# hritikbharucha/Custom_Porechop_ABI

Measured on AMD Instinct MI355X. Metric: reads/sec trimmed (100k ONT reads x 50 adapter pairs), higher is better.
Workload: dtype int32

## Files before the change

custom_porechop_abi_amd/csrc/pcabi_dp.h:

```cpp
#pragma once

#ifndef PCABI_ROW_FENCE
#define PCABI_ROW_FENCE 1
#endif
#ifndef PCABI_TAB_PD
#define PCABI_TAB_PD 0
#endif
#ifndef PCABI_TAB_PD_LONG
#define PCABI_TAB_PD_LONG 1
#endif

#include <stdint.h>
#include <algorithm>

#ifdef __HIPCC__
#define PCABI_HD __host__ __device__ __forceinline__
#else
#define PCABI_HD inline
#endif

namespace pcabi {

constexpr int NEG = -(1 << 28);

// ... 1158 lines not shown
template <typename TabRow>
struct ShiftRow {
    TabRow t;
    int32_t d;
    PCABI_HD int32_t operator()(int s) const { return addw(t(s), d); }
    PCABI_HD void quad(int q, int32_t *dst) const {
        t.quad(q, dst);
        for (int k = 0; k < 4; ++k) dst[k] = addw(dst[k], d);
    }
};
}

template <int RPL, int PD = PCABI_TAB_PD>
struct LaneShift {
    using Y = pk::LayS<RPL>;
    LanePacked<RPL, true, pk::LayT<RPL>, PD> st;
    int32_t kgo;
    int32_t ftop;
    int32_t k_e;
    int32_t k_eR;
    int32_t k_rb;
    int jj, P;

    PCABI_HD void init(int L, const Scoring &sc, int P_, int B) {
        using pk::addw;
        const int off = RPL - L;
        P = P_;
        jj = 0;
        k_e = Y::sc(-sc.ge);
        k_eR = Y::sc(-sc.ge * RPL);
        k_rb = Y::sc(sc.ge * P);
        ftop = Y::sc(-B);
        kgo = Y::sc(sc.go - sc.ge) + ((P - 1) << Y::TB_SH);
        int32_t fs = addw(ftop, kgo);
#pragma unroll
        for (int s = 1; s <= RPL; ++s) {
            fs = addw(fs, k_e);
            st.G[s] = addw(Y::start(off - s), fs);
            st.HK[s] = addw(fs, Y::sc(-1) + Y::TAG1);
        }
        st.bkey = Y::start(-L);
        st.bj = 0;
    }

    PCABI_HD void advance() {
        using pk::addw;
        ++jj;
        kgo -= Y::TAG1;
        ftop = addw(ftop, k_e);
        if (jj == P) {
            const int32_t rb = addw(k_rb, P << Y::TB_SH);
#pragma unroll
            for (int s = 1; s <= RPL; ++s) {
                st.G[s] = addw(st.G[s], rb);
                st.HK[s] = addw(st.HK[s], rb);
            }
            jj = 0;
            kgo += P << Y::TB_SH;
            ftop = addw(ftop, k_rb);
        }
    }

    template <typename TabRow>
    PCABI_HD void column(const TabRow &tab, const int j, const int off) {
        using pk::addw;
        const int32_t kg = vreg(kgo);
        const int32_t top = addw(ftop, kgo);
        int32_t gup = addw(Y::start(j + off), top);
        int32_t vup = Y::SENT;
        int32_t diag = addw(addw(Y::start(j - 1 + off), top), Y::TAG1 - k_e);
        constexpr int NQ = RPL / 4;
        int32_t t[RPL + 2];
// ... 6 lines not shown
#pragma unroll
        for (int s = 1; s <= RPL; ++s) {
            if (PD > 0 && (s & 3) == 1) {
                const int q = (s - 1) / 4 + PD + 1;
                if (q < NQ) tab.quad(q, t + 4 * q + 1);
            }
            int32_t diag_nx = 0;
            if (s < RPL) diag_nx = st.G[s] + (PD > 0 ? t[s + 1] : tab(s + 1));
            const int32_t hn = std::max(st.HK[s], st.G[s]);
            const int32_t vo = gup + Y::kv(s);
            const int32_t vn = std::max(vup, vo);
            const int32_t sn = max3i(diag, vn, hn);
            if (s == RPL) { lv = vn; ls = sn; }
            st.G[s] = (sn & ~Y::TAGM) + kg;
            st.HK[s] = hn;
            gup = st.G[s];
            vup = vn;
            diag = diag_nx;
#if defined(__HIP_DEVICE_COMPILE__)
            if (PCABI_ROW_FENCE > 0 && (s % (PCABI_ROW_FENCE > 0 ? PCABI_ROW_FENCE : 1)) == 0) __builtin_amdgcn_sched_barrier(0);
#endif
        }
        const int32_t corr = addw(std::max(lv, ls & ~Y::TAGM), pk::negw(addw(ftop, k_eR)));
        const bool upd = corr > (st.bkey | ((1 << Y::SC_SH) - 1));
        st.bkey = upd ? corr : st.bkey;
        st.bj = upd ? j : st.bj;
    }

    PCABI_HD void to_layt(const Scoring &sc) {
        using pk::addw;
        using pk::negw;
        const int32_t tagA = kgo - Y::sc(sc.go - sc.ge);
        int32_t cg = addw(negw(addw(ftop, kgo)), Y::sc(sc.go));
        int32_t ch = negw(addw(ftop, tagA + Y::TAG1));
#pragma unroll
        for (int s = 1; s <= RPL; ++s) {
            cg = addw(cg, negw(k_e));
            ch = addw(ch, negw(k_e));
            st.G[s] = addw(st.G[s], cg);
            st.HK[s] = addw(st.HK[s], ch);
        }
    }
};

template <int RPL, int PD = PCABI_TAB_PD, typename ReadFn, typename TabFn>
PCABI_HD Result align_lane_shift(ReadFn &rd, int n, const TabFn &tabfn, int L, const Scoring sc, int P, int B) {
    using Y = pk::LayS<RPL>;
    LaneShift<RPL, PD> ls;
    const int off = RPL - L;
    ls.init(L, sc, P, B);
    int r = rd(1);
#pragma unroll 1
    for (int j = 1; j < n; ++j) {
        const int rn = rd(j + 1);
        ls.advance();
        ls.template column<decltype(tabfn(r))>(tabfn(r), j, off);
        r = rn;
    }
    ls.to_layt(sc);
    auto &st = ls.st;
    const int32_t neg = Y::sc(pk::neg_score(sc));
    st.k_ge = vreg(Y::sc(sc.ge));
    st.k_go = vreg(Y::sc(sc.go));
    st.k_gev = st.k_geh = 0;
    st.k_gex = vreg(Y::sc(sc.ge) + Y::TB1);
    st.k_vo = Y::TB2;
    st.neg2 = neg | Y::TB2;
    st.materialize(L);
    const pk::ShiftRow<decltype(tabfn(r))> row{tabfn(r), Y::sc(sc.ge) + ((127 - Y::TDS) << Y::TB_SH)};
    st.template column<decltype(row), true>(row, n, L, off);
    Best b;
    b.score = st.bscore; b.bi = st.bi; b.bj = st.bj; b.attr = Y::to_std(st.battr, st.bj);
    b.ltype = st.blt; b.trail = st.btrail; b.precd = st.bprec;
    return finish(b, L, n);
}

template <int RPL, bool AFFINE, bool CHUNK = false, typename ReadFn, typename TabFn0, typename TabFn1>
PCABI_HD Result align_lane_packed_long(ReadFn &rd0, ReadFn &rd1, int n, const TabFn0 &tab0, const TabFn1 &tab1,
                                       int L, const Scoring sc, int own_lo = 1, int own_hi = -1) {
    int n_fin;
    Best b = packed_best<RPL, AFFINE, CHUNK, pk::LayL<RPL, 0>, PCABI_TAB_PD_LONG>(rd0, n, tab0, L, sc, own_lo, own_hi,
                                                                                 n_fin);
    const Best bm = packed_best<RPL, AFFINE, CHUNK, pk::LayL<RPL, 1>, PCABI_TAB_PD_LONG>(rd1, n, tab1, L, sc, own_lo,
                                                                                        own_hi, n_fin);
    b.attr |= bm.attr;
    return finish(b, L, n_fin);
}

struct SplitIn {
    int32_t gup, vup;
    int slt, vt, vp;
    int score, bi, lt, trail, prec;
    uint32_t attr;
};

template <int R, bool AFFINE, typename LAY>
struct LaneSplit {
// ... 352 lines not shown
```

custom_porechop_abi_amd/csrc/pcabi_kern.h:

```cpp
#pragma once
#include <hip/hip_runtime.h>

#include <algorithm>
#include <cstdint>
#include <cstdlib>
#include <string>
#include <type_traits>

#include "../../include/pcabi.h"
#include "pcabi_dp.h"

#ifndef PCABI_WAVES
#define PCABI_WAVES 1
#endif

void pcabi_poison(void *p, size_t bytes);
void pcabi_poison_async(void *p, size_t bytes, hipStream_t st);

namespace pcabi_eng {

int fail(int code, const std::string &msg);

#define HIP_TRY(expr)                                                                   \
    do {                                                                                \
// ... 131 lines not shown
        const int c = e / RPL, srow = e % RPL + 1;
        const uint32_t *ap = p.adp_pad + (int64_t)a_local * (RPL / 4);
        auto code = [&](int sl) { return (int)((ap[(sl - 1) / 4] >> (8 * ((sl - 1) & 3))) & 0xFFu); };
        wave_tab[e] = pcabi::pk::sub_key_shift<RPL>(srow, c, code, off, p.sc);
    }
    __syncthreads();
}

template <int RPL>
__device__ __forceinline__ void fill_wave_tab_long(const KParams &p, int a_local, int L, int32_t *wave_tab) {
    const int off = RPL - L;
    const int lane = threadIdx.x & 63;
    const uint32_t *ap = p.adp_pad + (int64_t)a_local * (RPL / 4);
    auto code = [&](int sl) { return (int)((ap[(sl - 1) / 4] >> (8 * ((sl - 1) & 3))) & 0xFFu); };
    for (int e = lane; e < kTabW * RPL; e += 64) {
        const int c = e / RPL, srow = e % RPL + 1;
        wave_tab[e] = pcabi::pk::sub_key<RPL, decltype(code), pcabi::pk::LayL<RPL, 0>>(srow, c, code, off, p.sc);
        wave_tab[kTabW * RPL + e] =
            pcabi::pk::sub_key<RPL, decltype(code), pcabi::pk::LayL<RPL, 1>>(srow, c, code, off, p.sc);
    }
    __syncthreads();
}

template <int RPL, bool AFFINE, int KIND>
__device__ __forceinline__ void run_lane(const KParams &p, int a_local, int64_t w, int64_t out_idx,
                                         int32_t *wave_tab, int64_t tile_off) {
    AdapterRegs<RPL> adp;
    if constexpr (KIND != LONG) adp.load(p.adp_pad + (int64_t)a_local * (RPL / 4));
    const int L = __builtin_amdgcn_readfirstlane(p.adp_len[a_local]);
    if constexpr (KIND == PACKED) fill_wave_tab<RPL>(p, a_local, L, wave_tab);
    if constexpr (KIND == TAGGED) fill_wave_tab<RPL, pcabi::pk::LayT<RPL>>(p, a_local, L, wave_tab);
    if constexpr (KIND == SHIFT) fill_wave_tab_shift<RPL>(p, a_local, L, wave_tab);
    if constexpr (KIND == LONG) fill_wave_tab_long<RPL>(p, a_local, L, wave_tab);
    if (w < 0) return;
    const int n = p.win_len[w];
    pcabi::Result r;
    if (n <= 0) {
        r = empty_result();
    } else {
        WindowReader rd = tile_off >= 0
            ? WindowReader(p.tiles + tile_off + (threadIdx.x & 255), 256, 0)
            : [&] {
                  const uint8_t *b = p.codes + p.win_off[w];
                  const int a0 = (int)((uintptr_t)b & 3);
                  return WindowReader(reinterpret_cast<const uint32_t *>(b - a0), 1, 8 * a0);
              }();
        if constexpr (KIND == PACKED) {
            auto tabfn = [&](int rc) { return LdsRow{wave_tab + rc * RPL}; };
            r = pcabi::align_lane_packed<(RPL <= pcabi::pk::MAX_RPL ? RPL : 4), AFFINE>(rd, n, tabfn, L, p.sc);
        } else if constexpr (KIND == TAGGED) {
            static_assert(RPL <= 32 && AFFINE, "run-tagged layout: affine buckets of <= 32 rows");
            auto tabfn = [&](int rc) { return LdsRow{wave_tab + rc * RPL}; };
            r = pcabi::align_lane_packed<RPL, true, false, pcabi::pk::LayT<RPL>>(rd, n, tabfn, L, p.sc);
        } else if constexpr (KIND == SHIFT) {
            static_assert(RPL <= 32 && AFFINE, "gap-extend frame: affine buckets of <= 32 rows");
            auto tabfn = [&](int rc) { return LdsRow{wave_tab + rc * RPL}; };
            r = pcabi::align_lane_shift<RPL>(rd, n, tabfn, L, p.sc, p.shift_p, p.shift_b);
        } else if constexpr (KIND == LONG) {
            WindowReader rd1 = rd;
            auto tab0 = [&](int rc) { return LdsRow{wave_tab + rc * RPL}; };
// ... 487 lines not shown
```

Baseline: 15.80 million.

## Add 4-column unrolled shift DP path for wave-uniform tiled windows

Adds align_lane_shift4, which reads one packed 32-bit tile word per four read columns and runs four DP columns per loop iteration. Only the first column of each group checks the periodic rebase; the other three use a cheaper step() since P is a multiple of 4. The fast path runs only when every lane in the wave has the same window length and tiled input, so per-column reader overhead and branches go away and loads are prefetched two words ahead. The best-score comparison is also changed to compare extracted scores, and the change adds register pressure and an extra wave-wide ballot check.

```diff
diff --git a/custom_porechop_abi_amd/csrc/pcabi_dp.h b/custom_porechop_abi_amd/csrc/pcabi_dp.h
--- a/custom_porechop_abi_amd/csrc/pcabi_dp.h
+++ b/custom_porechop_abi_amd/csrc/pcabi_dp.h
@@ -1204,16 +1204,16 @@
     int32_t k_rb;
     int jj, P;
 
-    PCABI_HD void init(int L, const Scoring &sc, int P_, int B) {
+    PCABI_HD void init(int L, const Scoring &sc, int P_, int B, int j0 = 0) {
         using pk::addw;
         const int off = RPL - L;
         P = P_;
-        jj = 0;
+        jj = j0;
         k_e = Y::sc(-sc.ge);
         k_eR = Y::sc(-sc.ge * RPL);
         k_rb = Y::sc(sc.ge * P);
-        ftop = Y::sc(-B);
-        kgo = Y::sc(sc.go - sc.ge) + ((P - 1) << Y::TB_SH);
+        ftop = Y::sc(-sc.ge * j0 - B);
+        kgo = Y::sc(sc.go - sc.ge) + ((P - 1 - j0) << Y::TB_SH);
         int32_t fs = addw(ftop, kgo);
 #pragma unroll
         for (int s = 1; s <= RPL; ++s) {
@@ -1225,11 +1225,15 @@
         st.bj = 0;
     }
 
+    PCABI_HD void step() {
+        ++jj;
+        kgo -= Y::TAG1;
+        ftop = pk::addw(ftop, k_e);
+    }
+
     PCABI_HD void advance() {
         using pk::addw;
-        ++jj;
-        kgo -= Y::TAG1;
-        ftop = addw(ftop, k_e);
+        step();
         if (jj == P) {
             const int32_t rb = addw(k_rb, P << Y::TB_SH);
 #pragma unroll
@@ -1282,7 +1286,7 @@
 #endif
         }
         const int32_t corr = addw(std::max(lv, ls & ~Y::TAGM), pk::negw(addw(ftop, k_eR)));
-        const bool upd = corr > (st.bkey | ((1 << Y::SC_SH) - 1));
+        const bool upd = Y::score(corr) > Y::score(st.bkey);
         st.bkey = upd ? corr : st.bkey;
         st.bj = upd ? j : st.bj;
     }
@@ -1303,9 +1307,29 @@
     }
 };
 
+template <int RPL, int PD, typename TabRow>
+PCABI_HD Result shift_last(LaneShift<RPL, PD> &ls, const TabRow &tab, int n, int L, const Scoring &sc) {
+    using Y = pk::LayS<RPL>;
+    ls.to_layt(sc);
+    auto &st = ls.st;
+    const int32_t neg = Y::sc(pk::neg_score(sc));
+    st.k_ge = vreg(Y::sc(sc.ge));
+    st.k_go = vreg(Y::sc(sc.go));
+    st.k_gev = st.k_geh = 0;
+    st.k_gex = vreg(Y::sc(sc.ge) + Y::TB1);
+    st.k_vo = Y::TB2;
+    st.neg2 = neg | Y::TB2;
+    st.materialize(L);
+    const pk::ShiftRow<TabRow> row{tab, Y::sc(sc.ge) + ((127 - Y::TDS) << Y::TB_SH)};
+    st.template column<decltype(row), true>(row, n, L, RPL - L);
+    Best b;
+    b.score = st.bscore; b.bi = st.bi; b.bj = st.bj; b.attr = Y::to_std(st.battr, st.bj);
+    b.ltype = st.blt; b.trail = st.btrail; b.precd = st.bprec;
+    return finish(b, L, n);
+}
+
 template <int RPL, int PD = PCABI_TAB_PD, typename ReadFn, typename TabFn>
 PCABI_HD Result align_lane_shift(ReadFn &rd, int n, const TabFn &tabfn, int L, const Scoring sc, int P, int B) {
-    using Y = pk::LayS<RPL>;
     LaneShift<RPL, PD> ls;
     const int off = RPL - L;
     ls.init(L, sc, P, B);
@@ -1317,22 +1341,37 @@
         ls.template column<decltype(tabfn(r))>(tabfn(r), j, off);
         r = rn;
     }
-    ls.to_layt(sc);
-    auto &st = ls.st;
-    const int32_t neg = Y::sc(pk::neg_score(sc));
-    st.k_ge = vreg(Y::sc(sc.ge));
-    st.k_go = vreg(Y::sc(sc.go));
-    st.k_gev = st.k_geh = 0;
-    st.k_gex = vreg(Y::sc(sc.ge) + Y::TB1);
-    st.k_vo = Y::TB2;
-    st.neg2 = neg | Y::TB2;
-    st.materialize(L);
-    const pk::ShiftRow<decltype(tabfn(r))> row{tabfn(r), Y::sc(sc.ge) + ((127 - Y::TDS) << Y::TB_SH)};
-    st.template column<decltype(row), true>(row, n, L, off);
-    Best b;
-    b.score = st.bscore; b.bi = st.bi; b.bj = st.bj; b.attr = Y::to_std(st.battr, st.bj);
-    b.ltype = st.blt; b.trail = st.btrail; b.precd = st.bprec;
-    return finish(b, L, n);
+    return shift_last<RPL, PD>(ls, tabfn(r), n, L, sc);
+}
+
+template <int RPL, int PD = PCABI_TAB_PD, typename TileFn, typename TabFn>
+PCABI_HD Result align_lane_shift4(const TileFn &tr, int n, const TabFn &tabfn, int L, const Scoring sc, int P, int B) {
+    LaneShift<RPL, PD> ls;
+    const int off = RPL - L;
+    ls.init(L, sc, P, B, -1);
+    const int np = (n - 1) / 4;
+    uint32_t cur = tr(0), nx = tr(1);
+    int j = 1;
+#pragma unroll 1
+    for (int q = 0; q < np; ++q, j += 4) {
+        const uint32_t w = cur;
+        cur = nx;
+        nx = tr(q + 2);
+        ls.advance();
+        ls.template column<decltype(tabfn(0))>(tabfn((int)(w & 0xFFu)), j, off);
+        ls.step();
+        ls.template column<decltype(tabfn(0))>(tabfn((int)((w >> 8) & 0xFFu)), j + 1, off);
+        ls.step();
+        ls.template column<decltype(tabfn(0))>(tabfn((int)((w >> 16) & 0xFFu)), j + 2, off);
+        ls.step();
+        ls.template column<decltype(tabfn(0))>(tabfn((int)(w >> 24)), j + 3, off);
+    }
+#pragma unroll 1
+    for (; j < n; ++j) {
+        ls.advance();
+        ls.template column<decltype(tabfn(0))>(tabfn((int)((cur >> (8 * ((j - 1) & 3))) & 0xFFu)), j, off);
+    }
+    return shift_last<RPL, PD>(ls, tabfn((int)((cur >> (8 * ((n - 1) & 3))) & 0xFFu)), n, L, sc);
 }
 
 template <int RPL, bool AFFINE, bool CHUNK = false, typename ReadFn, typename TabFn0, typename TabFn1>
diff --git a/custom_porechop_abi_amd/csrc/pcabi_kern.h b/custom_porechop_abi_amd/csrc/pcabi_kern.h
--- a/custom_porechop_abi_amd/csrc/pcabi_kern.h
+++ b/custom_porechop_abi_amd/csrc/pcabi_kern.h
@@ -177,6 +177,8 @@
     __syncthreads();
 }
 
+constexpr int kShift4MaxRows = 24;
+
 template <int RPL, bool AFFINE, int KIND>
 __device__ __forceinline__ void run_lane(const KParams &p, int a_local, int64_t w, int64_t out_idx,
                                          int32_t *wave_tab, int64_t tile_off) {
@@ -190,7 +192,20 @@
     if (w < 0) return;
     const int n = p.win_len[w];
     pcabi::Result r;
-    if (n <= 0) {
+    bool uniform = false;
+    if constexpr (KIND == SHIFT) {
+        const int n0 = __builtin_amdgcn_readfirstlane(n);
+        const int P = __builtin_amdgcn_readfirstlane(p.shift_p);
+        if (RPL <= kShift4MaxRows && n0 > 0 && (P & 3) == 0 && __builtin_amdgcn_ballot_w64(n != n0 || tile_off < 0) == 0) {
+            const uint32_t *base = p.tiles + tile_off + (threadIdx.x & 255);
+            auto tr = [&](int q) { return base[(int64_t)q * 256]; };
+            auto tabfn = [&](int rc) { return LdsRow{wave_tab + rc * RPL}; };
+            r = pcabi::align_lane_shift4<RPL>(tr, n0, tabfn, L, p.sc, P, p.shift_b);
+            uniform = true;
+        }
+    }
+    if (uniform) {
+    } else if (n <= 0) {
         r = empty_result();
     } else {
         WindowReader rd = tile_off >= 0
diff --git a/profiles/r08/k_align24_shift4_inner_pass.s b/profiles/r08/k_align24_shift4_inner_pass.s
--- /dev/null
+++ b/profiles/r08/k_align24_shift4_inner_pass.s
@@ -0,0 +1,1008 @@
+	s_mov_b64 s[4:5], 0x400
+.LBB5_25:
+	global_load_dword v62, v[8:9], off
+	s_add_i32 s53, s53, 1
+	s_add_i32 s48, s48, 0xfffe0000
+	s_add_i32 s47, s47, s42
+	s_cmp_lg_u32 s53, s34
+	s_cbranch_scc1 .LBB5_27
+	v_add_u32_e32 v59, s50, v59
+	v_add_u32_e32 v60, s50, v60
+	v_add_u32_e32 v57, s50, v57
+	v_add_u32_e32 v58, s50, v58
+	v_add_u32_e32 v55, s50, v55
+	v_add_u32_e32 v56, s50, v56
+	v_add_u32_e32 v53, s50, v53
+	v_add_u32_e32 v54, s50, v54
+	v_add_u32_e32 v51, s50, v51
+	v_add_u32_e32 v52, s50, v52
+	v_add_u32_e32 v49, s50, v49
+	v_add_u32_e32 v50, s50, v50
+	v_add_u32_e32 v47, s50, v47
+	v_add_u32_e32 v48, s50, v48
+	v_add_u32_e32 v45, s50, v45
+	v_add_u32_e32 v46, s50, v46
+	v_add_u32_e32 v43, s50, v43
+	v_add_u32_e32 v44, s50, v44
+	v_add_u32_e32 v41, s50, v41
+	v_add_u32_e32 v42, s50, v42
+	v_add_u32_e32 v39, s50, v39
+	v_add_u32_e32 v40, s50, v40
+	v_add_u32_e32 v37, s50, v37
+	v_add_u32_e32 v38, s50, v38
+	v_add_u32_e32 v35, s50, v35
+	v_add_u32_e32 v36, s50, v36
+	v_add_u32_e32 v33, s50, v33
+	v_add_u32_e32 v34, s50, v34
+	v_add_u32_e32 v31, s50, v31
+	v_add_u32_e32 v32, s50, v32
+	v_add_u32_e32 v29, s50, v29
+	v_add_u32_e32 v30, s50, v30
+	v_add_u32_e32 v27, s50, v27
+	v_add_u32_e32 v28, s50, v28
+	v_add_u32_e32 v25, s50, v25
+	v_add_u32_e32 v26, s50, v26
+	v_add_u32_e32 v23, s50, v23
+	v_add_u32_e32 v24, s50, v24
+	v_add_u32_e32 v20, s50, v20
+	v_add_u32_e32 v21, s50, v21
+	v_add_u32_e32 v17, s50, v17
+	v_add_u32_e32 v19, s50, v19
+	v_add_u32_e32 v15, s50, v15
+	v_add_u32_e32 v16, s50, v16
+	v_add_u32_e32 v22, s50, v22
+	v_add_u32_e32 v14, s50, v14
+	v_add_u32_e32 v10, s50, v10
+	v_add_u32_e32 v11, s50, v11
+	s_add_i32 s48, s48, s45
+	s_add_i32 s47, s47, s44
+	s_mov_b32 s53, 0
+.LBB5_27:
+	s_waitcnt vmcnt(2)
+	v_and_b32_e32 v63, 0xff, v61
+	v_mad_u32_u24 v63, v63, s52, v18
+	v_mov_b32_e32 v66, s48
+	s_add_i32 s36, s51, 0xfffff400
+	ds_read_b64 v[64:65], v63
+	s_and_b32 s36, s36, 0x1fc00
+	s_add_i32 s10, s47, s48
+	s_add_i32 s11, s51, 0xfffdf800
+	s_sub_i32 s36, s36, s42
+	s_and_b32 s11, s11, 0x1fc00
+	s_add_i32 s36, s10, s36
+	s_add_i32 s36, s36, 0x20000
+	s_add_i32 s10, s10, s11
+	s_waitcnt lgkmcnt(0)
+	v_add_u32_e32 v64, s36, v64
+	v_add_u32_e32 v65, v65, v59
+	v_max_i32_e32 v59, v60, v59
+	s_add_i32 s10, s10, 0xbe0000
+	v_max3_i32 v60, v64, s10, v59
+	v_and_b32_e32 v60, 0xff01ffff, v60
+	v_add_u32_e32 v60, v60, v66
+	ds_read_b32 v64, v63 offset:8
+	v_add_u32_e32 v67, 0xbc0000, v60
+	v_max_i32_e32 v58, v58, v57
+	v_max_i32_e32 v67, s10, v67
+	v_max3_i32 v65, v65, v67, v58
+	s_waitcnt lgkmcnt(0)
+	v_add_u32_e32 v57, v64, v57
+	v_and_b32_e32 v64, 0xff01ffff, v65
+	v_add_u32_e32 v64, v64, v66
+	ds_read_b32 v65, v63 offset:12
+	v_add_u32_e32 v68, 0xba0000, v64
+	v_max_i32_e32 v56, v56, v55
+	v_max_i32_e32 v67, v67, v68
+	v_max3_i32 v57, v57, v67, v56
+	v_and_b32_e32 v57, 0xff01ffff, v57
+	s_waitcnt lgkmcnt(0)
+	v_add_u32_e32 v55, v65, v55
+	v_add_u32_e32 v57, v57, v66
+	ds_read_b32 v65, v63 offset:16
+	v_add_u32_e32 v68, 0xb80000, v57
+	v_max_i32_e32 v54, v54, v53
+	v_max_i32_e32 v67, v67, v68
+	v_max3_i32 v55, v55, v67, v54
+	v_and_b32_e32 v55, 0xff01ffff, v55
+	s_waitcnt lgkmcnt(0)
+	v_add_u32_e32 v53, v65, v53
+	v_add_u32_e32 v55, v55, v66
+	ds_read_b32 v65, v63 offset:20
+	v_add_u32_e32 v68, 0xb60000, v55
+	v_max_i32_e32 v52, v52, v51
+	v_max_i32_e32 v67, v67, v68
+	v_max3_i32 v53, v53, v67, v52
+	v_and_b32_e32 v53, 0xff01ffff, v53
+	s_waitcnt lgkmcnt(0)
+	v_add_u32_e32 v51, v65, v51
+	v_add_u32_e32 v53, v53, v66
+	ds_read_b32 v65, v63 offset:24
+	v_add_u32_e32 v68, 0xb40000, v53
+	v_max_i32_e32 v50, v50, v49
+	v_max_i32_e32 v67, v67, v68
+	v_max3_i32 v51, v51, v67, v50
+	v_and_b32_e32 v51, 0xff01ffff, v51
+	s_waitcnt lgkmcnt(0)
+	v_add_u32_e32 v49, v65, v49
+	v_add_u32_e32 v51, v51, v66
+	ds_read_b32 v65, v63 offset:28
+	v_add_u32_e32 v68, 0xb20000, v51
+	v_max_i32_e32 v48, v48, v47
+	v_max_i32_e32 v67, v67, v68
+	v_max3_i32 v49, v49, v67, v48
+	v_and_b32_e32 v49, 0xff01ffff, v49
+	s_waitcnt lgkmcnt(0)
+	v_add_u32_e32 v47, v65, v47
+	v_add_u32_e32 v49, v49, v66
+	ds_read_b32 v65, v63 offset:32
+	v_add_u32_e32 v68, 0xb00000, v49
+	v_max_i32_e32 v46, v46, v45
+	v_max_i32_e32 v67, v67, v68
+	v_max3_i32 v47, v47, v67, v46
+	v_and_b32_e32 v47, 0xff01ffff, v47
+	s_waitcnt lgkmcnt(0)
+	v_add_u32_e32 v45, v65, v45
+	v_add_u32_e32 v47, v47, v66
+	ds_read_b32 v65, v63 offset:36
+	v_add_u32_e32 v68, 0xae0000, v47
+	v_max_i32_e32 v44, v44, v43
+	v_max_i32_e32 v67, v67, v68
+	v_max3_i32 v45, v45, v67, v44
+	v_and_b32_e32 v45, 0xff01ffff, v45
+	s_waitcnt lgkmcnt(0)
+	v_add_u32_e32 v43, v65, v43
+	v_add_u32_e32 v45, v45, v66
+	ds_read_b32 v65, v63 offset:40
+	v_add_u32_e32 v68, 0xac0000, v45
+	v_max_i32_e32 v42, v42, v41
+	v_max_i32_e32 v67, v67, v68
+	v_max3_i32 v43, v43, v67, v42
+	v_and_b32_e32 v43, 0xff01ffff, v43
+	s_waitcnt lgkmcnt(0)
+	v_add_u32_e32 v41, v65, v41
+	v_add_u32_e32 v43, v43, v66
+	ds_read_b32 v65, v63 offset:44
+	v_add_u32_e32 v68, 0xaa0000, v43
+	v_max_i32_e32 v40, v40, v39
+	v_max_i32_e32 v67, v67, v68
+	v_max3_i32 v41, v41, v67, v40
+	v_and_b32_e32 v41, 0xff01ffff, v41
+	s_waitcnt lgkmcnt(0)
+	v_add_u32_e32 v39, v65, v39
+	v_add_u32_e32 v41, v41, v66
+	ds_read_b32 v65, v63 offset:48
+	v_add_u32_e32 v68, 0xa80000, v41
+	v_max_i32_e32 v38, v38, v37
+	v_max_i32_e32 v67, v67, v68
+	v_max3_i32 v39, v39, v67, v38
+	v_and_b32_e32 v39, 0xff01ffff, v39
+	s_waitcnt lgkmcnt(0)
+	v_add_u32_e32 v37, v65, v37
+	v_add_u32_e32 v39, v39, v66
+	ds_read_b32 v65, v63 offset:52
+	v_add_u32_e32 v68, 0xa60000, v39
+	v_max_i32_e32 v36, v36, v35
+	v_max_i32_e32 v67, v67, v68
+	v_max3_i32 v37, v37, v67, v36
+	v_and_b32_e32 v37, 0xff01ffff, v37
+	s_waitcnt lgkmcnt(0)
+	v_add_u32_e32 v35, v65, v35
+	v_add_u32_e32 v37, v37, v66
+	ds_read_b32 v65, v63 offset:56
+	v_add_u32_e32 v68, 0xa40000, v37
+	v_max_i32_e32 v34, v34, v33
+	v_max_i32_e32 v67, v67, v68
+	v_max3_i32 v35, v35, v67, v34
+	v_and_b32_e32 v35, 0xff01ffff, v35
+	s_waitcnt lgkmcnt(0)
+	v_add_u32_e32 v33, v65, v33
+	v_add_u32_e32 v35, v35, v66
+	ds_read_b32 v65, v63 offset:60
+	v_add_u32_e32 v68, 0xa20000, v35
+	v_max_i32_e32 v32, v32, v31
+	v_max_i32_e32 v67, v67, v68
+	v_max3_i32 v33, v33, v67, v32
+	v_and_b32_e32 v33, 0xff01ffff, v33
+	s_waitcnt lgkmcnt(0)
+	v_add_u32_e32 v31, v65, v31
+	v_add_u32_e32 v33, v33, v66
+	ds_read_b32 v65, v63 offset:64
+	v_add_u32_e32 v68, 0xa00000, v33
+	v_max_i32_e32 v30, v30, v29
+	v_max_i32_e32 v67, v67, v68
+	v_max3_i32 v31, v31, v67, v30
+	v_and_b32_e32 v31, 0xff01ffff, v31
+	s_waitcnt lgkmcnt(0)
+	v_add_u32_e32 v29, v65, v29
+	v_add_u32_e32 v31, v31, v66
+	ds_read_b32 v65, v63 offset:68
+	v_add_u32_e32 v68, 0x9e0000, v31
+	v_max_i32_e32 v28, v28, v27
+	v_max_i32_e32 v67, v67, v68
+	v_max3_i32 v29, v29, v67, v28
+	v_and_b32_e32 v29, 0xff01ffff, v29
+	s_waitcnt lgkmcnt(0)
+	v_add_u32_e32 v27, v65, v27
+	v_add_u32_e32 v29, v29, v66
+	ds_read_b32 v65, v63 offset:72
+	v_add_u32_e32 v68, 0x9c0000, v29
+	v_max_i32_e32 v26, v26, v25
+	v_max_i32_e32 v67, v67, v68
+	v_max3_i32 v27, v27, v67, v26
+	v_and_b32_e32 v27, 0xff01ffff, v27
+	s_waitcnt lgkmcnt(0)
+	v_add_u32_e32 v25, v65, v25
+	v_add_u32_e32 v27, v27, v66
+	ds_read_b32 v65, v63 offset:76
+	v_add_u32_e32 v68, 0x9a0000, v27
+	v_max_i32_e32 v24, v24, v23
+	v_max_i32_e32 v67, v67, v68
+	v_max3_i32 v25, v25, v67, v24
+	v_and_b32_e32 v25, 0xff01ffff, v25
+	s_waitcnt lgkmcnt(0)
+	v_add_u32_e32 v23, v65, v23
+	v_add_u32_e32 v25, v25, v66
+	ds_read_b32 v65, v63 offset:80
+	v_add_u32_e32 v68, 0x980000, v25
+	v_max_i32_e32 v21, v21, v20
+	v_max_i32_e32 v67, v67, v68
+	v_max3_i32 v23, v23, v67, v21
+	v_and_b32_e32 v23, 0xff01ffff, v23
+	s_waitcnt lgkmcnt(0)
+	v_add_u32_e32 v20, v65, v20
+	v_add_u32_e32 v23, v23, v66
+	ds_read_b32 v65, v63 offset:84
+	v_add_u32_e32 v68, 0x960000, v23
+	v_max_i32_e32 v19, v19, v17
+	v_max_i32_e32 v67, v67, v68
+	v_max3_i32 v20, v20, v67, v19
+	v_and_b32_e32 v20, 0xff01ffff, v20
+	s_waitcnt lgkmcnt(0)
+	v_add_u32_e32 v17, v65, v17
+	v_add_u32_e32 v20, v20, v66
+	ds_read_b32 v65, v63 offset:88
+	v_add_u32_e32 v68, 0x940000, v20
+	v_max_i32_e32 v16, v16, v15
+	v_max_i32_e32 v67, v67, v68
+	v_max3_i32 v17, v17, v67, v16
+	v_and_b32_e32 v17, 0xff01ffff, v17
+	s_waitcnt lgkmcnt(0)
+	v_add_u32_e32 v15, v65, v15
+	v_add_u32_e32 v17, v17, v66
+	v_add_u32_e32 v65, 0x920000, v17
+	ds_read_b32 v63, v63 offset:92
+	v_max_i32_e32 v14, v14, v22
+	v_max_i32_e32 v65, v67, v65
+	v_max3_i32 v15, v15, v65, v14
+	v_and_b32_e32 v15, 0xff01ffff, v15
+	v_add_u32_e32 v15, v15, v66
+	s_waitcnt lgkmcnt(0)
+	v_add_u32_e32 v22, v63, v22
+	v_max_i32_e32 v63, v11, v10
+	v_add_u32_e32 v10, 0x900000, v15
+	v_max_i32_e32 v10, v65, v10
+	v_max3_i32 v11, v22, v10, v63
+	v_and_b32_e32 v11, 0xff01ffff, v11
+	v_add_u32_e32 v22, v11, v66
+	v_max_i32_e32 v10, v10, v11
+	s_sub_i32 s10, s43, s47
+	v_add_u32_e32 v10, s10, v10
+	v_cmp_gt_i32_sdwa vcc, sext(v10), sext(v13) src0_sel:BYTE_3 src1_sel:BYTE_3
+	s_add_i32 s10, s48, 0xfffe0000
+	v_mov_b32_e32 v66, s10
+	v_cndmask_b32_e32 v13, v13, v10, vcc
+	v_mov_b32_e32 v10, s9
+	v_cndmask_b32_e32 v7, v7, v10, vcc
+	v_bfe_u32 v10, v61, 8, 8
+	v_mad_u32_u24 v65, v10, s52, v18
+	s_add_i32 s36, s51, 0xfffff800
+	ds_read_b64 v[10:11], v65
+	s_add_i32 s47, s47, s42
+	s_and_b32 s36, s36, 0x1fc00
+	s_add_i32 s10, s47, s10
+	s_add_i32 s11, s51, 0xfffdfc00
+	s_sub_i32 s36, s36, s42
+	s_and_b32 s11, s11, 0x1fc00
+	s_add_i32 s36, s10, s36
+	s_add_i32 s36, s36, 0x20000
+	s_add_i32 s10, s10, s11
+	s_waitcnt lgkmcnt(0)
+	v_add_u32_e32 v10, s36, v10
+	v_max_i32_e32 v59, v59, v60
+	s_add_i32 s10, s10, 0xbe0000
+	v_max3_i32 v10, v10, s10, v59
+	v_and_b32_e32 v10, 0xff01ffff, v10
+	v_add_u32_e32 v11, v11, v60
+	v_add_u32_e32 v60, v10, v66
+	ds_read_b32 v10, v65 offset:8
+	v_add_u32_e32 v67, 0xbc0000, v60
+	v_max_i32_e32 v58, v58, v64
+	v_max_i32_e32 v67, s10, v67
+	v_max3_i32 v11, v11, v67, v58
+	s_waitcnt lgkmcnt(0)
+	v_add_u32_e32 v10, v10, v64
+	v_and_b32_e32 v11, 0xff01ffff, v11
+	v_add_u32_e32 v64, v11, v66
+	ds_read_b32 v11, v65 offset:12
+	v_add_u32_e32 v68, 0xba0000, v64
+	v_max_i32_e32 v56, v56, v57
+	v_max_i32_e32 v67, v67, v68
+	v_max3_i32 v10, v10, v67, v56
+	v_and_b32_e32 v10, 0xff01ffff, v10
+	s_waitcnt lgkmcnt(0)
+	v_add_u32_e32 v11, v11, v57
+	v_add_u32_e32 v57, v10, v66
+	ds_read_b32 v10, v65 offset:16
+	v_add_u32_e32 v68, 0xb80000, v57
+	v_max_i32_e32 v54, v54, v55
+	v_max_i32_e32 v67, v67, v68
+	v_max3_i32 v11, v11, v67, v54
+	v_and_b32_e32 v11, 0xff01ffff, v11
+	s_waitcnt lgkmcnt(0)
+	v_add_u32_e32 v10, v10, v55
+	v_add_u32_e32 v55, v11, v66
+	ds_read_b32 v11, v65 offset:20
+	v_add_u32_e32 v68, 0xb60000, v55
+	v_max_i32_e32 v52, v52, v53
+	v_max_i32_e32 v67, v67, v68
+	v_max3_i32 v10, v10, v67, v52
+	v_and_b32_e32 v10, 0xff01ffff, v10
+	s_waitcnt lgkmcnt(0)
+	v_add_u32_e32 v11, v11, v53
+	v_add_u32_e32 v53, v10, v66
+	ds_read_b32 v10, v65 offset:24
+	v_add_u32_e32 v68, 0xb40000, v53
+	v_max_i32_e32 v50, v50, v51
+	v_max_i32_e32 v67, v67, v68
+	v_max3_i32 v11, v11, v67, v50
+	v_and_b32_e32 v11, 0xff01ffff, v11
+	s_waitcnt lgkmcnt(0)
+	v_add_u32_e32 v10, v10, v51
+	v_add_u32_e32 v51, v11, v66
+	ds_read_b32 v11, v65 offset:28
+	v_add_u32_e32 v68, 0xb20000, v51
+	v_max_i32_e32 v48, v48, v49
+	v_max_i32_e32 v67, v67, v68
+	v_max3_i32 v10, v10, v67, v48
+	v_and_b32_e32 v10, 0xff01ffff, v10
+	s_waitcnt lgkmcnt(0)
+	v_add_u32_e32 v11, v11, v49
+	v_add_u32_e32 v49, v10, v66
+	ds_read_b32 v10, v65 offset:32
+	v_add_u32_e32 v68, 0xb00000, v49
+	v_max_i32_e32 v46, v46, v47
+	v_max_i32_e32 v67, v67, v68
+	v_max3_i32 v11, v11, v67, v46
+	v_and_b32_e32 v11, 0xff01ffff, v11
+	s_waitcnt lgkmcnt(0)
+	v_add_u32_e32 v10, v10, v47
+	v_add_u32_e32 v47, v11, v66
+	ds_read_b32 v11, v65 offset:36
+	v_add_u32_e32 v68, 0xae0000, v47
+	v_max_i32_e32 v44, v44, v45
+	v_max_i32_e32 v67, v67, v68
+	v_max3_i32 v10, v10, v67, v44
+	v_and_b32_e32 v10, 0xff01ffff, v10
+	s_waitcnt lgkmcnt(0)
+	v_add_u32_e32 v11, v11, v45
+	v_add_u32_e32 v45, v10, v66
+	ds_read_b32 v10, v65 offset:40
+	v_add_u32_e32 v68, 0xac0000, v45
+	v_max_i32_e32 v42, v42, v43
+	v_max_i32_e32 v67, v67, v68
+	v_max3_i32 v11, v11, v67, v42
+	v_and_b32_e32 v11, 0xff01ffff, v11
+	s_waitcnt lgkmcnt(0)
+	v_add_u32_e32 v10, v10, v43
+	v_add_u32_e32 v43, v11, v66
+	ds_read_b32 v11, v65 offset:44
+	v_add_u32_e32 v68, 0xaa0000, v43
+	v_max_i32_e32 v40, v40, v41
+	v_max_i32_e32 v67, v67, v68
+	v_max3_i32 v10, v10, v67, v40
+	v_and_b32_e32 v10, 0xff01ffff, v10
+	s_waitcnt lgkmcnt(0)
+	v_add_u32_e32 v11, v11, v41
+	v_add_u32_e32 v41, v10, v66
+	ds_read_b32 v10, v65 offset:48
+	v_add_u32_e32 v68, 0xa80000, v41
+	v_max_i32_e32 v38, v38, v39
+	v_max_i32_e32 v67, v67, v68
+	v_max3_i32 v11, v11, v67, v38
+	v_and_b32_e32 v11, 0xff01ffff, v11
+	s_waitcnt lgkmcnt(0)
+	v_add_u32_e32 v10, v10, v39
+	v_add_u32_e32 v39, v11, v66
+	ds_read_b32 v11, v65 offset:52
+	v_add_u32_e32 v68, 0xa60000, v39
+	v_max_i32_e32 v36, v36, v37
+	v_max_i32_e32 v67, v67, v68
+	v_max3_i32 v10, v10, v67, v36
+	v_and_b32_e32 v10, 0xff01ffff, v10
+	s_waitcnt lgkmcnt(0)
+	v_add_u32_e32 v11, v37, v11
+	v_add_u32_e32 v37, v10, v66
+	ds_read_b32 v10, v65 offset:56
+	v_add_u32_e32 v68, 0xa40000, v37
+	v_max_i32_e32 v34, v34, v35
+	v_max_i32_e32 v67, v67, v68
+	v_max3_i32 v11, v11, v67, v34
+	v_and_b32_e32 v11, 0xff01ffff, v11
+	s_waitcnt lgkmcnt(0)
+	v_add_u32_e32 v10, v35, v10
+	v_add_u32_e32 v35, v11, v66
+	ds_read_b32 v11, v65 offset:60
+	v_add_u32_e32 v68, 0xa20000, v35
+	v_max_i32_e32 v32, v32, v33
+	v_max_i32_e32 v67, v67, v68
+	v_max3_i32 v10, v10, v67, v32
+	v_and_b32_e32 v10, 0xff01ffff, v10
+	s_waitcnt lgkmcnt(0)
+	v_add_u32_e32 v11, v33, v11
+	v_add_u32_e32 v33, v10, v66
+	ds_read_b32 v10, v65 offset:64
+	v_add_u32_e32 v68, 0xa00000, v33
+	v_max_i32_e32 v30, v30, v31
+	v_max_i32_e32 v67, v67, v68
+	v_max3_i32 v11, v11, v67, v30
+	v_and_b32_e32 v11, 0xff01ffff, v11
+	s_waitcnt lgkmcnt(0)
+	v_add_u32_e32 v10, v31, v10
+	v_add_u32_e32 v31, v11, v66
+	ds_read_b32 v11, v65 offset:68
+	v_add_u32_e32 v68, 0x9e0000, v31
+	v_max_i32_e32 v28, v28, v29
+	v_max_i32_e32 v67, v67, v68
+	v_max3_i32 v10, v10, v67, v28
+	v_and_b32_e32 v10, 0xff01ffff, v10
+	s_waitcnt lgkmcnt(0)
+	v_add_u32_e32 v11, v29, v11
+	v_add_u32_e32 v29, v10, v66
+	ds_read_b32 v10, v65 offset:72
+	v_add_u32_e32 v68, 0x9c0000, v29
+	v_max_i32_e32 v26, v26, v27
+	v_max_i32_e32 v67, v67, v68
+	v_max3_i32 v11, v11, v67, v26
+	v_and_b32_e32 v11, 0xff01ffff, v11
+	s_waitcnt lgkmcnt(0)
+	v_add_u32_e32 v10, v27, v10
+	v_add_u32_e32 v27, v11, v66
+	ds_read_b32 v11, v65 offset:76
+	v_add_u32_e32 v68, 0x9a0000, v27
+	v_max_i32_e32 v24, v24, v25
+	v_max_i32_e32 v67, v67, v68
+	v_max3_i32 v10, v10, v67, v24
+	v_and_b32_e32 v10, 0xff01ffff, v10
+	s_waitcnt lgkmcnt(0)
+	v_add_u32_e32 v11, v25, v11
+	v_add_u32_e32 v25, v10, v66
+	ds_read_b32 v10, v65 offset:80
+	v_add_u32_e32 v68, 0x980000, v25
+	v_max_i32_e32 v21, v21, v23
+	v_max_i32_e32 v67, v67, v68
+	v_max3_i32 v11, v11, v67, v21
+	v_and_b32_e32 v11, 0xff01ffff, v11
+	s_waitcnt lgkmcnt(0)
+	v_add_u32_e32 v10, v23, v10
+	v_add_u32_e32 v23, v11, v66
+	ds_read_b32 v11, v65 offset:84
+	v_add_u32_e32 v68, 0x960000, v23
+	v_max_i32_e32 v19, v19, v20
+	v_max_i32_e32 v67, v67, v68
+	v_max3_i32 v10, v10, v67, v19
+	v_and_b32_e32 v10, 0xff01ffff, v10
+	s_waitcnt lgkmcnt(0)
+	v_add_u32_e32 v11, v20, v11
+	v_add_u32_e32 v20, v10, v66
+	ds_read_b32 v10, v65 offset:88
+	v_add_u32_e32 v68, 0x940000, v20
+	v_max_i32_e32 v16, v16, v17
+	v_max_i32_e32 v67, v67, v68
+	v_max3_i32 v11, v11, v67, v16
+	v_and_b32_e32 v11, 0xff01ffff, v11
+	s_waitcnt lgkmcnt(0)
+	v_add_u32_e32 v10, v17, v10
+	v_add_u32_e32 v17, v11, v66
+	ds_read_b32 v11, v65 offset:92
+	v_add_u32_e32 v65, 0x920000, v17
+	v_max_i32_e32 v14, v14, v15
+	v_max_i32_e32 v65, v67, v65
+	v_max3_i32 v10, v10, v65, v14
+	v_and_b32_e32 v10, 0xff01ffff, v10
+	v_add_u32_e32 v67, v10, v66
+	s_waitcnt lgkmcnt(0)
+	v_add_u32_e32 v10, v15, v11
+	v_add_u32_e32 v11, 0x900000, v67
+	v_max_i32_e32 v15, v63, v22
+	v_max_i32_e32 v11, v65, v11
+	v_max3_i32 v10, v10, v11, v15
+	v_and_b32_e32 v10, 0xff01ffff, v10
+	v_add_u32_e32 v22, v10, v66
+	v_max_i32_e32 v10, v11, v10
+	s_sub_i32 s10, s43, s47
+	v_add_u32_e32 v10, s10, v10
+	v_cmp_gt_i32_sdwa vcc, sext(v10), sext(v13) src0_sel:BYTE_3 src1_sel:BYTE_3
+	s_add_i32 s10, s9, 1
+	s_add_i32 s36, s51, 0xfffffc00
+	v_cndmask_b32_e32 v13, v13, v10, vcc
+	v_mov_b32_e32 v10, s10
+	v_cndmask_b32_e32 v7, v7, v10, vcc
+	s_add_i32 s10, s48, 0xfffc0000
+	v_bfe_u32 v10, v61, 16, 8
+	v_mad_u32_u24 v63, v10, s52, v18
+	v_mov_b32_e32 v65, s10
+	ds_read_b64 v[10:11], v63
+	s_add_i32 s47, s47, s42
+	s_and_b32 s36, s36, 0x1fc00
+	s_add_i32 s10, s47, s10
+	s_add_i32 s11, s51, 0xfffe0000
+	s_sub_i32 s36, s36, s42
+	s_and_b32 s11, s11, 0x1fc00
+	s_add_i32 s36, s10, s36
+	s_add_i32 s36, s36, 0x20000
+	s_add_i32 s10, s10, s11
+	s_waitcnt lgkmcnt(0)
+	v_add_u32_e32 v10, s36, v10
+	v_max_i32_e32 v59, v59, v60
+	s_add_i32 s10, s10, 0xbe0000
+	v_max3_i32 v10, v10, s10, v59
+	v_and_b32_e32 v10, 0xff01ffff, v10
+	v_add_u32_e32 v11, v11, v60
+	v_add_u32_e32 v60, v10, v65
+	ds_read_b32 v10, v63 offset:8
+	v_add_u32_e32 v66, 0xbc0000, v60
+	v_max_i32_e32 v58, v58, v64
+	v_max_i32_e32 v66, s10, v66
+	v_max3_i32 v11, v11, v66, v58
+	s_waitcnt lgkmcnt(0)
+	v_add_u32_e32 v10, v10, v64
+	v_and_b32_e32 v11, 0xff01ffff, v11
+	v_add_u32_e32 v64, v11, v65
+	ds_read_b32 v11, v63 offset:12
+	v_add_u32_e32 v68, 0xba0000, v64
+	v_max_i32_e32 v56, v56, v57
+	v_max_i32_e32 v66, v66, v68
+	v_max3_i32 v10, v10, v66, v56
+	s_waitcnt lgkmcnt(0)
+	v_add_u32_e32 v11, v11, v57
+	v_and_b32_e32 v10, 0xff01ffff, v10
+	v_add_u32_e32 v68, v10, v65
+	ds_read_b32 v10, v63 offset:16
+	v_add_u32_e32 v57, 0xb80000, v68
+	v_max_i32_e32 v54, v54, v55
+	v_max_i32_e32 v57, v66, v57
+	v_max3_i32 v11, v11, v57, v54
+	s_waitcnt lgkmcnt(0)
+	v_add_u32_e32 v10, v10, v55
+	v_and_b32_e32 v11, 0xff01ffff, v11
+	v_add_u32_e32 v66, v11, v65
+	ds_read_b32 v11, v63 offset:20
+	v_add_u32_e32 v55, 0xb60000, v66
+	v_max_i32_e32 v52, v52, v53
+	v_max_i32_e32 v55, v57, v55
+	v_max3_i32 v10, v10, v55, v52
+	s_waitcnt lgkmcnt(0)
+	v_add_u32_e32 v11, v11, v53
+	v_and_b32_e32 v10, 0xff01ffff, v10
+	v_add_u32_e32 v69, v10, v65
+	ds_read_b32 v10, v63 offset:24
+	v_add_u32_e32 v53, 0xb40000, v69
+	v_max_i32_e32 v50, v50, v51
+	v_max_i32_e32 v53, v55, v53
+	v_max3_i32 v11, v11, v53, v50
+	s_waitcnt lgkmcnt(0)
+	v_add_u32_e32 v10, v10, v51
+	v_and_b32_e32 v11, 0xff01ffff, v11
+	v_add_u32_e32 v70, v11, v65
+	ds_read_b32 v11, v63 offset:28
+	v_add_u32_e32 v51, 0xb20000, v70
+	v_max_i32_e32 v48, v48, v49
+	v_max_i32_e32 v51, v53, v51
+	v_max3_i32 v10, v10, v51, v48
+	s_waitcnt lgkmcnt(0)
+	v_add_u32_e32 v11, v11, v49
+	v_and_b32_e32 v10, 0xff01ffff, v10
+	v_add_u32_e32 v71, v10, v65
+	ds_read_b32 v10, v63 offset:32
+	v_add_u32_e32 v49, 0xb00000, v71
+	v_max_i32_e32 v46, v46, v47
+	v_max_i32_e32 v49, v51, v49
+	v_max3_i32 v11, v11, v49, v46
+	s_waitcnt lgkmcnt(0)
+	v_add_u32_e32 v10, v10, v47
+	v_and_b32_e32 v11, 0xff01ffff, v11
+	v_add_u32_e32 v72, v11, v65
+	ds_read_b32 v11, v63 offset:36
+	v_add_u32_e32 v47, 0xae0000, v72
+	v_max_i32_e32 v44, v44, v45
+	v_max_i32_e32 v47, v49, v47
+	v_max3_i32 v10, v10, v47, v44
+	s_waitcnt lgkmcnt(0)
+	v_add_u32_e32 v11, v11, v45
+	v_and_b32_e32 v10, 0xff01ffff, v10
+	v_add_u32_e32 v73, v10, v65
+	ds_read_b32 v10, v63 offset:40
+	v_add_u32_e32 v45, 0xac0000, v73
+	v_max_i32_e32 v42, v42, v43
+	v_max_i32_e32 v45, v47, v45
+	v_max3_i32 v11, v11, v45, v42
+	s_waitcnt lgkmcnt(0)
+	v_add_u32_e32 v10, v10, v43
+	v_and_b32_e32 v11, 0xff01ffff, v11
+	v_add_u32_e32 v74, v11, v65
+	ds_read_b32 v11, v63 offset:44
+	v_add_u32_e32 v43, 0xaa0000, v74
+	v_max_i32_e32 v40, v40, v41
+	v_max_i32_e32 v43, v45, v43
+	v_max3_i32 v10, v10, v43, v40
+	s_waitcnt lgkmcnt(0)
+	v_add_u32_e32 v11, v11, v41
+	v_and_b32_e32 v10, 0xff01ffff, v10
+	v_add_u32_e32 v75, v10, v65
+	ds_read_b32 v10, v63 offset:48
+	v_add_u32_e32 v41, 0xa80000, v75
+	v_max_i32_e32 v38, v38, v39
+	v_max_i32_e32 v41, v43, v41
+	v_max3_i32 v11, v11, v41, v38
+	s_waitcnt lgkmcnt(0)
+	v_add_u32_e32 v10, v10, v39
+	v_and_b32_e32 v11, 0xff01ffff, v11
+	v_add_u32_e32 v76, v11, v65
+	ds_read_b32 v11, v63 offset:52
+	v_add_u32_e32 v39, 0xa60000, v76
+	v_max_i32_e32 v36, v36, v37
+	v_max_i32_e32 v39, v41, v39
+	v_max3_i32 v10, v10, v39, v36
+	s_waitcnt lgkmcnt(0)
+	v_add_u32_e32 v11, v37, v11
+	v_and_b32_e32 v10, 0xff01ffff, v10
+	v_add_u32_e32 v77, v10, v65
+	ds_read_b32 v10, v63 offset:56
+	v_add_u32_e32 v37, 0xa40000, v77
+	v_max_i32_e32 v34, v34, v35
+	v_max_i32_e32 v37, v39, v37
+	v_max3_i32 v11, v11, v37, v34
+	s_waitcnt lgkmcnt(0)
+	v_add_u32_e32 v10, v35, v10
+	v_and_b32_e32 v11, 0xff01ffff, v11
+	v_add_u32_e32 v78, v11, v65
+	ds_read_b32 v11, v63 offset:60
+	v_add_u32_e32 v35, 0xa20000, v78
+	v_max_i32_e32 v32, v32, v33
+	v_max_i32_e32 v35, v37, v35
+	v_max3_i32 v10, v10, v35, v32
+	s_waitcnt lgkmcnt(0)
+	v_add_u32_e32 v11, v33, v11
+	v_and_b32_e32 v10, 0xff01ffff, v10
+	v_add_u32_e32 v79, v10, v65
+	ds_read_b32 v10, v63 offset:64
+	v_add_u32_e32 v33, 0xa00000, v79
+	v_max_i32_e32 v30, v30, v31
+	v_max_i32_e32 v33, v35, v33
+	v_max3_i32 v11, v11, v33, v30
+	s_waitcnt lgkmcnt(0)
+	v_add_u32_e32 v10, v31, v10
+	v_and_b32_e32 v11, 0xff01ffff, v11
+	v_add_u32_e32 v80, v11, v65
+	ds_read_b32 v11, v63 offset:68
+	v_add_u32_e32 v31, 0x9e0000, v80
+	v_max_i32_e32 v28, v28, v29
+	v_max_i32_e32 v31, v33, v31
+	v_max3_i32 v10, v10, v31, v28
+	s_waitcnt lgkmcnt(0)
+	v_add_u32_e32 v11, v29, v11
+	v_and_b32_e32 v10, 0xff01ffff, v10
+	v_add_u32_e32 v81, v10, v65
+	ds_read_b32 v10, v63 offset:72
+	v_add_u32_e32 v29, 0x9c0000, v81
+	v_max_i32_e32 v26, v26, v27
+	v_max_i32_e32 v29, v31, v29
+	v_max3_i32 v11, v11, v29, v26
+	s_waitcnt lgkmcnt(0)
+	v_add_u32_e32 v10, v27, v10
+	v_and_b32_e32 v11, 0xff01ffff, v11
+	v_add_u32_e32 v82, v11, v65
+	ds_read_b32 v11, v63 offset:76
+	v_add_u32_e32 v27, 0x9a0000, v82
+	v_max_i32_e32 v24, v24, v25
+	v_max_i32_e32 v27, v29, v27
+	v_max3_i32 v10, v10, v27, v24
+	s_waitcnt lgkmcnt(0)
+	v_add_u32_e32 v11, v25, v11
+	v_and_b32_e32 v10, 0xff01ffff, v10
+	v_add_u32_e32 v83, v10, v65
+	ds_read_b32 v10, v63 offset:80
+	v_add_u32_e32 v25, 0x980000, v83
+	v_max_i32_e32 v21, v21, v23
+	v_max_i32_e32 v25, v27, v25
+	v_max3_i32 v11, v11, v25, v21
+	s_waitcnt lgkmcnt(0)
+	v_add_u32_e32 v10, v23, v10
+	v_and_b32_e32 v11, 0xff01ffff, v11
+	v_add_u32_e32 v84, v11, v65
+	ds_read_b32 v11, v63 offset:84
+	v_add_u32_e32 v23, 0x960000, v84
+	v_max_i32_e32 v19, v19, v20
+	v_max_i32_e32 v23, v25, v23
+	v_max3_i32 v10, v10, v23, v19
+	s_waitcnt lgkmcnt(0)
+	v_add_u32_e32 v11, v20, v11
+	v_and_b32_e32 v10, 0xff01ffff, v10
+	v_add_u32_e32 v85, v10, v65
+	ds_read_b32 v10, v63 offset:88
+	v_add_u32_e32 v20, 0x940000, v85
+	v_max_i32_e32 v16, v16, v17
+	v_max_i32_e32 v20, v23, v20
+	v_max3_i32 v11, v11, v20, v16
+	s_waitcnt lgkmcnt(0)
+	v_add_u32_e32 v10, v17, v10
+	v_and_b32_e32 v11, 0xff01ffff, v11
+	v_add_u32_e32 v86, v11, v65
+	ds_read_b32 v11, v63 offset:92
+	v_add_u32_e32 v17, 0x920000, v86
+	v_max_i32_e32 v14, v14, v67
+	v_max_i32_e32 v17, v20, v17
+	v_max3_i32 v10, v10, v17, v14
+	v_and_b32_e32 v10, 0xff01ffff, v10
+	v_add_u32_e32 v63, v10, v65
+	s_waitcnt lgkmcnt(0)
+	v_add_u32_e32 v10, v67, v11
+	v_add_u32_e32 v11, 0x900000, v63
+	v_max_i32_e32 v67, v15, v22
+	v_max_i32_e32 v11, v17, v11
+	v_max3_i32 v10, v10, v11, v67
+	v_and_b32_e32 v10, 0xff01ffff, v10
+	v_add_u32_e32 v65, v10, v65
+	v_max_i32_e32 v10, v11, v10
+	s_sub_i32 s10, s43, s47
+	v_add_u32_e32 v10, s10, v10
+	v_cmp_gt_i32_sdwa vcc, sext(v10), sext(v13) src0_sel:BYTE_3 src1_sel:BYTE_3
+	s_add_i32 s10, s9, 2
+	s_add_i32 s48, s48, 0xfffa0000
+	v_cndmask_b32_e32 v13, v13, v10, vcc
+	v_mov_b32_e32 v10, s10
+	v_cndmask_b32_e32 v7, v7, v10, vcc
+	v_lshrrev_b32_e32 v10, 24, v61
+	v_mad_u32_u24 v22, v10, s52, v18
+	v_mov_b32_e32 v61, s48
+	ds_read_b64 v[10:11], v22
+	s_add_i32 s47, s47, s42
+	s_and_b32 s36, s51, 0x1fc00
+	s_add_i32 s10, s47, s48
+	s_add_i32 s11, s51, 0xfffe0400
+	s_sub_i32 s36, s36, s42
+	s_and_b32 s11, s11, 0x1fc00
+	s_add_i32 s36, s10, s36
+	s_add_i32 s36, s36, 0x20000
+	s_add_i32 s10, s10, s11
+	s_waitcnt lgkmcnt(0)
+	v_add_u32_e32 v10, s36, v10
+	v_add_u32_e32 v11, v11, v60
+	v_max_i32_e32 v60, v59, v60
+	s_add_i32 s10, s10, 0xbe0000
+	v_max3_i32 v10, v10, s10, v60
+	v_and_b32_e32 v10, 0xff01ffff, v10
+	s_add_i32 s53, s53, 3
+	v_add_u32_e32 v59, v10, v61
+	ds_read_b32 v10, v22 offset:8
+	v_add_u32_e32 v15, 0xbc0000, v59
+	v_max_i32_e32 v58, v58, v64
+	v_max_i32_e32 v15, s10, v15
+	v_max3_i32 v11, v11, v15, v58
+	v_and_b32_e32 v11, 0xff01ffff, v11
+	s_waitcnt lgkmcnt(0)
+	v_add_u32_e32 v10, v10, v64
+	v_add_u32_e32 v57, v11, v61
+	ds_read_b32 v11, v22 offset:12
+	v_add_u32_e32 v17, 0xba0000, v57
+	v_max_i32_e32 v56, v56, v68
+	v_max_i32_e32 v15, v15, v17
+	v_max3_i32 v10, v10, v15, v56
+	v_and_b32_e32 v10, 0xff01ffff, v10
+	s_waitcnt lgkmcnt(0)
+	v_add_u32_e32 v11, v11, v68
+	v_add_u32_e32 v55, v10, v61
+	ds_read_b32 v10, v22 offset:16
+	v_add_u32_e32 v17, 0xb80000, v55
+	v_max_i32_e32 v54, v54, v66
+	v_max_i32_e32 v15, v15, v17
+	v_max3_i32 v11, v11, v15, v54
+	v_and_b32_e32 v11, 0xff01ffff, v11
+	s_waitcnt lgkmcnt(0)
+	v_add_u32_e32 v10, v10, v66
+	v_add_u32_e32 v53, v11, v61
+	ds_read_b32 v11, v22 offset:20
+	v_add_u32_e32 v17, 0xb60000, v53
+	v_max_i32_e32 v52, v52, v69
+	v_max_i32_e32 v15, v15, v17
+	v_max3_i32 v10, v10, v15, v52
+	v_and_b32_e32 v10, 0xff01ffff, v10
+	s_waitcnt lgkmcnt(0)
+	v_add_u32_e32 v11, v11, v69
+	v_add_u32_e32 v51, v10, v61
+	ds_read_b32 v10, v22 offset:24
+	v_add_u32_e32 v17, 0xb40000, v51
+	v_max_i32_e32 v50, v50, v70
+	v_max_i32_e32 v15, v15, v17
+	v_max3_i32 v11, v11, v15, v50
+	v_and_b32_e32 v11, 0xff01ffff, v11
+	s_waitcnt lgkmcnt(0)
+	v_add_u32_e32 v10, v10, v70
+	v_add_u32_e32 v49, v11, v61
+	ds_read_b32 v11, v22 offset:28
+	v_add_u32_e32 v17, 0xb20000, v49
+	v_max_i32_e32 v48, v48, v71
+	v_max_i32_e32 v15, v15, v17
+	v_max3_i32 v10, v10, v15, v48
+	v_and_b32_e32 v10, 0xff01ffff, v10
+	s_waitcnt lgkmcnt(0)
+	v_add_u32_e32 v11, v11, v71
+	v_add_u32_e32 v47, v10, v61
+	ds_read_b32 v10, v22 offset:32
+	v_add_u32_e32 v17, 0xb00000, v47
+	v_max_i32_e32 v46, v46, v72
+	v_max_i32_e32 v15, v15, v17
+	v_max3_i32 v11, v11, v15, v46
+	v_and_b32_e32 v11, 0xff01ffff, v11
+	s_waitcnt lgkmcnt(0)
+	v_add_u32_e32 v10, v10, v72
+	v_add_u32_e32 v45, v11, v61
+	ds_read_b32 v11, v22 offset:36
+	v_add_u32_e32 v17, 0xae0000, v45
+	v_max_i32_e32 v44, v44, v73
+	v_max_i32_e32 v15, v15, v17
+	v_max3_i32 v10, v10, v15, v44
+	v_and_b32_e32 v10, 0xff01ffff, v10
+	s_waitcnt lgkmcnt(0)
+	v_add_u32_e32 v11, v11, v73
+	v_add_u32_e32 v43, v10, v61
+	ds_read_b32 v10, v22 offset:40
+	v_add_u32_e32 v17, 0xac0000, v43
+	v_max_i32_e32 v42, v42, v74
+	v_max_i32_e32 v15, v15, v17
+	v_max3_i32 v11, v11, v15, v42
+	v_and_b32_e32 v11, 0xff01ffff, v11
+	s_waitcnt lgkmcnt(0)
+	v_add_u32_e32 v10, v10, v74
+	v_add_u32_e32 v41, v11, v61
+	ds_read_b32 v11, v22 offset:44
+	v_add_u32_e32 v17, 0xaa0000, v41
+	v_max_i32_e32 v40, v40, v75
+	v_max_i32_e32 v15, v15, v17
+	v_max3_i32 v10, v10, v15, v40
+	v_and_b32_e32 v10, 0xff01ffff, v10
+	s_waitcnt lgkmcnt(0)
+	v_add_u32_e32 v11, v11, v75
+	v_add_u32_e32 v39, v10, v61
+	ds_read_b32 v10, v22 offset:48
+	v_add_u32_e32 v17, 0xa80000, v39
+	v_max_i32_e32 v38, v38, v76
+	v_max_i32_e32 v15, v15, v17
+	v_max3_i32 v11, v11, v15, v38
+	v_and_b32_e32 v11, 0xff01ffff, v11
+	s_waitcnt lgkmcnt(0)
+	v_add_u32_e32 v10, v10, v76
+	v_add_u32_e32 v37, v11, v61
+	ds_read_b32 v11, v22 offset:52
+	v_add_u32_e32 v17, 0xa60000, v37
+	v_max_i32_e32 v36, v36, v77
+	v_max_i32_e32 v15, v15, v17
+	v_max3_i32 v10, v10, v15, v36
+	v_and_b32_e32 v10, 0xff01ffff, v10
+	s_waitcnt lgkmcnt(0)
+	v_add_u32_e32 v11, v77, v11
+	v_add_u32_e32 v35, v10, v61
+	ds_read_b32 v10, v22 offset:56
+	v_add_u32_e32 v17, 0xa40000, v35
+	v_max_i32_e32 v34, v34, v78
+	v_max_i32_e32 v15, v15, v17
+	v_max3_i32 v11, v11, v15, v34
+	v_and_b32_e32 v11, 0xff01ffff, v11
+	s_waitcnt lgkmcnt(0)
+	v_add_u32_e32 v10, v78, v10
+	v_add_u32_e32 v33, v11, v61
+	ds_read_b32 v11, v22 offset:60
+	v_add_u32_e32 v17, 0xa20000, v33
+	v_max_i32_e32 v32, v32, v79
+	v_max_i32_e32 v15, v15, v17
+	v_max3_i32 v10, v10, v15, v32
+	v_and_b32_e32 v10, 0xff01ffff, v10
+	s_waitcnt lgkmcnt(0)
+	v_add_u32_e32 v11, v79, v11
+	v_add_u32_e32 v31, v10, v61
+	ds_read_b32 v10, v22 offset:64
+	v_add_u32_e32 v17, 0xa00000, v31
+	v_max_i32_e32 v30, v30, v80
+	v_max_i32_e32 v15, v15, v17
+	v_max3_i32 v11, v11, v15, v30
+	v_and_b32_e32 v11, 0xff01ffff, v11
+	s_waitcnt lgkmcnt(0)
+	v_add_u32_e32 v10, v80, v10
+	v_add_u32_e32 v29, v11, v61
+	ds_read_b32 v11, v22 offset:68
+	v_add_u32_e32 v17, 0x9e0000, v29
+	v_max_i32_e32 v28, v28, v81
+	v_max_i32_e32 v15, v15, v17
+	v_max3_i32 v10, v10, v15, v28
+	v_and_b32_e32 v10, 0xff01ffff, v10
+	s_waitcnt lgkmcnt(0)
+	v_add_u32_e32 v11, v81, v11
+	v_add_u32_e32 v27, v10, v61
+	ds_read_b32 v10, v22 offset:72
+	v_add_u32_e32 v17, 0x9c0000, v27
+	v_max_i32_e32 v26, v26, v82
+	v_max_i32_e32 v15, v15, v17
+	v_max3_i32 v11, v11, v15, v26
+	v_and_b32_e32 v11, 0xff01ffff, v11
+	s_waitcnt lgkmcnt(0)
+	v_add_u32_e32 v10, v82, v10
+	v_add_u32_e32 v25, v11, v61
+	ds_read_b32 v11, v22 offset:76
+	v_add_u32_e32 v17, 0x9a0000, v25
+	v_max_i32_e32 v24, v24, v83
+	v_max_i32_e32 v15, v15, v17
+	v_max3_i32 v10, v10, v15, v24
+	v_and_b32_e32 v10, 0xff01ffff, v10
+	s_waitcnt lgkmcnt(0)
+	v_add_u32_e32 v11, v83, v11
+	v_add_u32_e32 v23, v10, v61
+	ds_read_b32 v10, v22 offset:80
+	v_add_u32_e32 v17, 0x980000, v23
+	v_max_i32_e32 v21, v21, v84
+	v_max_i32_e32 v15, v15, v17
+	v_max3_i32 v11, v11, v15, v21
+	v_and_b32_e32 v11, 0xff01ffff, v11
+	s_waitcnt lgkmcnt(0)
+	v_add_u32_e32 v10, v84, v10
+	v_add_u32_e32 v20, v11, v61
+	ds_read_b32 v11, v22 offset:84
+	v_add_u32_e32 v17, 0x960000, v20
+	v_max_i32_e32 v19, v19, v85
+	v_max_i32_e32 v15, v15, v17
+	v_max3_i32 v10, v10, v15, v19
+	v_and_b32_e32 v10, 0xff01ffff, v10
+	s_waitcnt lgkmcnt(0)
+	v_add_u32_e32 v11, v85, v11
+	v_add_u32_e32 v17, v10, v61
+	ds_read_b32 v10, v22 offset:88
+	v_add_u32_e32 v64, 0x940000, v17
+	v_max_i32_e32 v16, v16, v86
+	v_max_i32_e32 v64, v15, v64
+	v_max3_i32 v11, v11, v64, v16
+	v_and_b32_e32 v11, 0xff01ffff, v11
+	s_waitcnt lgkmcnt(0)
+	v_add_u32_e32 v10, v86, v10
+	v_add_u32_e32 v15, v11, v61
+	ds_read_b32 v11, v22 offset:92
+	v_add_u32_e32 v22, 0x920000, v15
+	v_max_i32_e32 v14, v14, v63
+	v_max_i32_e32 v64, v64, v22
+	v_max3_i32 v10, v10, v64, v14
+	v_and_b32_e32 v10, 0xff01ffff, v10
+	v_add_u32_e32 v22, v10, v61
+	s_waitcnt lgkmcnt(0)
+	v_add_u32_e32 v10, v63, v11
+	v_add_u32_e32 v63, 0x900000, v22
+	v_max_i32_e32 v11, v67, v65
+	v_max_i32_e32 v63, v64, v63
+	v_max3_i32 v10, v10, v63, v11
+	v_and_b32_e32 v64, 0xff01ffff, v10
+	v_add_u32_e32 v10, v64, v61
+	v_max_i32_e32 v61, v63, v64
+	s_sub_i32 s10, s43, s47
+	v_add_u32_e32 v61, s10, v61
+	v_cmp_gt_i32_sdwa vcc, sext(v61), sext(v13) src0_sel:BYTE_3 src1_sel:BYTE_3
+	s_add_i32 s10, s9, 3
+	s_add_i32 s9, s9, 4
+	v_cndmask_b32_e32 v13, v13, v61, vcc
+	v_mov_b32_e32 v61, s10
+	s_add_i32 s49, s49, -1
+	s_addk_i32 s51, 0x1000
+	v_cndmask_b32_e32 v7, v7, v61, vcc
+	s_cmp_eq_u32 s49, 0
+	v_lshl_add_u64 v[8:9], v[8:9], 0, s[4:5]
+	s_cbranch_scc1 .LBB5_30
+	s_waitcnt vmcnt(1)
+	v_mov_b32_e32 v61, v6
+	s_waitcnt vmcnt(0)
+	v_mov_b32_e32 v6, v62
```

After: 16.18 million, median of 6. +2.4%, better.
